# thiery-lab/manifold-mcmc-for-diffusions

Measured on AMD Instinct MI355X. Metric: constrained-leapfrog steps/sec (all chains), FHN noisy-obs 400 sub-steps, higher is better.
Workload: dtype f64; 1 GPU; FHN noisy-obs, T=100 obs, S=400 steps/obs, R=5 obs/subseq, sigma_y=0.1, 256 chains per GPU (BASELINE.json configs[1]), Newton solver, standard splitting; chains_per_gpu=256, global_chains=256, dim_q=80106, traj_len=16, stepping=chmc_leapfrog_steps per trajectory (batched steps), chain_steps_nominal=152320, parallelism=chains x1 (no data-path collective, 1 gather), ranks_joined=1, collective_world_size=1, collective_route=torch.distributed gather, overlap_halves=-1

## Files before the change

### manifold_mcmc_for_diffusions_amd/context.py

```python
import ctypes as C
import numpy as np
from . import _lib
from ._lib import ChmcConfig, as_c, ptr, iptr, check

MODEL_IDS = {"fhn": 0, "sir": 1, "fhn_nb": 2}
STATUS_NAMES = {0: "ok", 1: "not_converged", 2: "diverged", 3: "non_reversible", -1: "inactive"}


class ChmcContext:
    def __init__(self, model, obs_interval, num_steps_per_obs, num_obs_per_subseq, y_seq, sigma=None,
                 use_gaussian_splitting=False, num_chains=1, device=0):
        L = _lib.lib()
        self.L = L
        y = as_c(np.asarray(y_seq).reshape(-1))
        self._y = y
        cfg = ChmcConfig(
            model=MODEL_IDS[model] if isinstance(model, str) else int(model), num_obs=len(y),
            num_steps_per_obs=int(num_steps_per_obs),
            num_obs_per_subseq=0 if num_obs_per_subseq is None else int(num_obs_per_subseq),
            noisy=2 if isinstance(sigma, str) else int(sigma is not None),
            use_gaussian_splitting=int(bool(use_gaussian_splitting)),
            num_chains=int(num_chains), device=int(device), obs_interval=float(obs_interval),
            sigma=0.0 if sigma is None or isinstance(sigma, str) else float(sigma), y_seq=ptr(y))
        h = C.c_void_p()
# ... 317 lines not shown
                                         constraint_tol, position_tol, divergence_tol, int(max_iters), reverse_check_tol,
                                         iptr(ndone), iptr(status), iptr(itf), iptr(itb), ptr(rev)), "chmc_leapfrog_steps")
        return dict(n_done=ndone, status=status, iters_fwd=itf, iters_bwd=itb, rev_err=rev)

    def comm_init(self, id128, rank, world):
        buf = (C.c_char * 128).from_buffer_copy(bytes(id128))
        check(self.L.chmc_comm_init(self.h, buf, int(rank), int(world)), "chmc_comm_init")
        self.comm_world = int(world)

    @staticmethod
    def comm_unique_id():
        buf = (C.c_char * 128)()
        check(_lib.lib().chmc_comm_unique_id(buf), "chmc_comm_unique_id")
        return bytes(buf)

    def gather_samples_device(self, local_dev_ptr, count, gathered_dev_ptr):
        check(self.L.chmc_gather_samples(self.h, C.c_void_p(local_dev_ptr), int(count), C.c_void_p(gathered_dev_ptr)),
              "chmc_gather_samples")

    def comm_info(self):
        wd, rk = C.c_int(0), C.c_int(0)
        check(self.L.chmc_comm_info(self.h, C.byref(wd), C.byref(rk)), "chmc_comm_info")
        return wd.value, rk.value

    def comm_destroy(self):
        check(self.L.chmc_comm_destroy(self.h), "chmc_comm_destroy")

    def diagnostics(self):
        out = (C.c_longlong * 80)()
        check(self.L.chmc_get_diagnostics(self.h, out), "chmc_get_diagnostics")
        v = np.array(out[:], dtype=np.int64)
        return dict(par_scan=v[:64], gram_mfma_launches=int(v[64]), gram_valu_launches=int(v[65]),
                    retract_kernel_launches=int(v[66]), traj_kernel_launches=int(v[67]),
                    newton_fsm_launches=int(v[68]), newton_factor8_launches=int(v[69]), extra=v[68:80])

    def counters(self):
        out = (C.c_longlong * 8)()
        check(self.L.chmc_get_counters(self.h, out), "chmc_get_counters")
        keys = ("constr", "jacob_constr_blocks", "lu_jacob_product_blocks", "chol_gram_blocks",
                "grad_log_det_sqrt_gram", "leapfrog_step", "projection_iterations", "_")
        return dict(zip(keys, (int(v) for v in out)))
```

### manifold_mcmc_for_diffusions_amd/csrc/chmc_api.inc

```
#include <string>
#include <algorithm>
#include <vector>
#include <cstring>
#include <cstdio>
#include <cstdlib>
#include <cmath>
#include <thread>
#include <type_traits>
#include "../../include/chmc.h"
#include "chmc_plan.h"
#include "chmc_layout.h"

using namespace chmc;

static thread_local std::string g_err;
static int fail(const std::string& m) {
  g_err = m;
  return -1;
}
#include CHMC_BACKEND_HEADER

struct chmc_ctx : ChainView {
  std::thread::id owner = std::this_thread::get_id();
  chmc_config cfg;
// ... 572 lines not shown
    else
      launch_wave(k_jw_wave<RM>, (long)sy.B * sy.K, 6, sy, c->sl, c->w, which, vsel | 256);
#else
    launch(KJw<RM>{sy, c->sl, c->w, which, vsel | 256}, (long)sy.B * sy.K * RM, 6);
#endif
    launch(KSymBlk<M, RM>{sy, c->sl, c->w, which, 0}, (long)sy.B * sy.K, 9);
    CHMC_SOLVE_CHAIN(M, RM, 1, 1, sy, c->sl, c->w, which, 0, psel);
    if (compact) {
      CHMC_UPDATE_PB(1, which, 0, psel);
    } else {
      CHMC_UPDATE(1, sy, c->sl, c->w, which, 0, psel);
    }
  });
}

static void iteration_scan(chmc_ctx* c, int newton, int prev, int qsel, int fwd_guess, int use_nw) {
  const Sys& sy = c->sy;
  CHMC_DISPATCH(c, {
    if (newton) {
#ifdef CHMC_WAVE_KERNELS
      CHMC_FWD(prev ^ 1, qsel, use_nw, 2, fwd_guess);
#else
      (void)fwd_guess, (void)use_nw;
#endif
    } else {
      CHMC_FWD(prev ^ 1, qsel, use_nw, 0, fwd_guess);
    }
  });
}
static void iteration_after_scan(chmc_ctx* c, int newton, int prev, int qsel) {
  const Sys& sy = c->sy;
  const NewtonSweep sweep = part_plan(c).newton;
  const bool solved = newton && (sweep == NewtonIvlFsm || sweep == Newton16IvlCombFactor || sweep == Newton16IvlCombWg);
  CHMC_DISPATCH(c, {
    if (newton) {
#ifdef CHMC_WAVE_KERNELS
      const long nbk = (long)sy.B * sy.K;
      if constexpr (RM > 8) {
        switch (sweep) {
          case Newton16IvlCombWg:
            launch_blocks(k_newton_ivl<M>, nbk * sy.NOBS, 64, 1, sy, c->sl, c->w, prev, qsel);
            launch_blocks(k_newton_comb_wg<M, RM, CHMC_RETRACT_WAVES, false>, (long)sy.B, 64 * CHMC_RETRACT_WAVES, 1, sy,
                          c->sl, c->w, prev, qsel);
            break;
          case Newton16IvlCombFactor:
            launch_blocks(k_newton_ivl<M>, nbk * sy.NOBS, 64, 1, sy, c->sl, c->w, prev, qsel);
            launch_blocks(k_newton_comb<M, RM, false, true>, nbk, 64, 1, sy, c->sl, c->w, prev, qsel);
            break;
          case Newton16IvlComb:
            launch_blocks(k_newton_ivl<M>, nbk * sy.NOBS, 64, 1, sy, c->sl, c->w, prev, qsel);
            launch_blocks(k_newton_comb<M, RM>, nbk, 64, 1, sy, c->sl, c->w, prev, qsel);
            break;
          case Newton16LdsrowsGramMfma:
            launch_blocks(k_rev_wave_ldsrows<M, RM, 1>, nbk, 64, 1, sy, c->sl, c->w, prev, qsel);
            launch_blocks(k_gram_rows_mfma<RM>, nbk, 64, 1, sy, c->sl, c->w, prev, 1, qsel), c->diag[0]++;
            break;
          default:
            launch_blocks(k_rev_wave_ldsrows<M, RM, 1>, nbk, 64, 1, sy, c->sl, c->w, prev, qsel);
            launch_wave(k_gram_rows<RM, 4>, nbk * (RM / 4), 1, sy, c->sl, c->w, prev, 1, qsel), c->diag[1]++;
        }
        if (!solved) launch_blocks(k_newton_factor_wave<M, RM>, (nbk + 3) / 4, 64, 9, sy, c->sl, c->w, prev, qsel);
      } else {
        switch (sweep) {
          case NewtonIvlFsm:
          case NewtonIvlComb:
            launch_blocks(k_newton_ivl<M>, nbk * sy.NOBS, 64, 1, sy, c->sl, c->w, prev, qsel);
            launch_blocks(k_newton_comb<M, RM>, nbk, 64, 1, sy, c->sl, c->w, prev, qsel);
            break;
          case NewtonRevStoreGramMfma:
            launch_wave(k_rev_wave<M, RM, 1, false>, nbk, 1, sy, c->sl, c->w, prev, qsel);
            launch_blocks(k_gram_rows_mfma<RM>, nbk, 64, 1, sy, c->sl, c->w, prev, 1, qsel), c->diag[0]++;
            break;
          default:
            launch_wave(k_rev_wave<M, RM, 1>, nbk, 1, sy, c->sl, c->w, prev, qsel);
        }
        if (solved)
          launch_blocks(k_newton_fsm_wave<M, RM>, (long)sy.B, 64, 5, sy, c->sl, c->w, prev, qsel), c->diag[4]++;
        else
          launch(KNewtonFactor<M, RM>{sy, c->sl, c->w, prev}, nbk, 9), c->diag[5]++;
      }
#else
      launch(KNewtonBlk<M, RM>{sy, c->sl, c->w, prev, qsel}, (long)sy.B * sy.K, 1);
#endif
      if (!solved) CHMC_SOLVE_CHAIN(M, RM, 0, 0, sy, c->sl, c->w, prev, qsel, 0);
    } else {
      launch(KSymBlk<M, RM>{sy, c->sl, c->w, prev, 1}, (long)sy.B * sy.K, 9);
      CHMC_SOLVE_CHAIN(M, RM, 1, 0, sy, c->sl, c->w, prev, qsel, 0);
    }
#ifdef CHMC_WAVE_KERNELS
    if (c->plan.rows == RowsCompact) {
      if (!solved) launch(KMuF<RM, M::X, 0>{sy, c->sl, c->w, prev}, (long)sy.B * sy.K * sy.NOBS * M::X, 5);
      launch_colmax(KUpdatePB<RM, M::X, M::V, 0, 1>{sy, c->sl, c->w, prev, qsel, 0},
                    sy.T * sy.S + sy.V0 + (sy.noisy ? sy.T : 0), sy.B, 4);
    } else
#endif
    CHMC_UPDATE(0, sy, c->sl, c->w, prev, qsel, 0);
  });
}

static int retract_waves(const chmc_ctx* c, int newton, const void* views) {
  return chain_kernel_waves(c->plan, part_plan(c).retract_chain, c->sy.B, c->num_cus, newton != 0, views != nullptr);
}
static int traj_waves(const chmc_ctx* c, int n_inner, int newton) {
  const bool eligible = part_plan(c).traj_chain && n_inner == 1 && c->mom_tangent && c->halves == 1;
  return chain_kernel_waves(c->plan, eligible, c->sy.B, c->num_cus, newton != 0, false);
}
static int run_projection(chmc_ctx* c, int newton, int prev, int qsel, double ctol, double ptol, double dtol,
                          int max_iters, const ViewSave* views = nullptr, int count_dir = -1) {
  const Sys& sy = c->sy;
#ifdef CHMC_WAVE_KERNELS
  if (const int waves = retract_waves(c, newton, views)) {
    int* iters_dst = count_dir < 0 ? nullptr : (count_dir ? c->d_itb : c->d_itf);
    CHMC_DISPATCH(c, {
      if constexpr (RM == 16) {
        if (waves == 4)
          launch_blocks(k_retract_chain<M, RM, 4>, (long)sy.B, 256, 1, sy, c->sl, c->w, prev, qsel, ctol, ptol, dtol, max_iters,
                        iters_dst);
        else
          launch_blocks(k_retract_chain<M, RM, CHMC_RETRACT_WAVES>, (long)sy.B, 64 * CHMC_RETRACT_WAVES, 1, sy, c->sl, c->w, prev,
                        qsel, ctol, ptol, dtol, max_iters, iters_dst);
      }
    });
    c->counters[6]++;
    c->diag[2]++;
    return 0;
  }
#endif
  const int nh = views ? 2 : 1;
  auto enter = [&](int h) {
    if (views) set_half(c, *views, h);
  };
  for (int h = 0; h < nh; ++h) {
    enter(h);
    if (sy.B > 0) launch(KNewtonBegin{c->w}, sy.B);
  }
  int fwd_guess = 2;
#ifdef CHMC_WAVE_KERNELS
  const bool carry = c->plan.par_scan && sy.K == 1;
#else
  const bool carry = false;
#endif
  const int max_rounds = carry ? 12 * (max_iters + 1) : max_iters;
  auto iteration = [&](int poll_slot) {
    iteration_scan(c, newton, prev, qsel, fwd_guess, 1);
    iteration_after_scan(c, newton, prev, qsel);
    const KCheck chk{c->w, ctol, ptol, dtol, max_iters, sy.B, count_dir < 0 ? nullptr : (count_dir ? c->d_itb : c->d_itf),
                     c->round & 3};
    if (poll_slot >= 0) launch_publish(chk, sy.B, c->w.n_active + (c->round & 3), poll_slot);
    else launch(chk, sy.B);
  };
  bool done[2] = {false, nh == 1};
  for (int h = 0; h < nh; ++h) {
    enter(h);
    if (sy.B <= 0) done[h] = true;
  }
  int& expect = c->proj_rounds[prev & 1];
  int& stable = c->proj_stable[prev & 1];
  const bool predict = !views && stable >= 3 && expect >= 2;
  int rounds_done = 0;
  for (int it = 0; it < max_rounds && !(done[0] && done[1]); ++it) {
    if (predict && it >= expect && poll_end((it - 1) & 1) == 0) {
      done[0] = true;
      break;
    }
    for (int h = 0; h < nh; ++h) {
      if (done[h]) continue;
      enter(h);
      fwd_guess = it == 0 ? 2 : 1;
      c->round = it;
      iteration(it >= 1 ? 2 * h + (it & 1) : -1);
    }
    c->counters[6]++;
    if (it == 0) continue;
    bool all_empty = true;
    for (int h = 0; h < nh; ++h) {
      if (done[h]) continue;
      if (it >= 2 && poll_end(2 * h + ((it - 1) & 1)) == 0) {
        done[h] = true;
        continue;
      }
      all_empty = false;
      if (it + 1 >= max_rounds) poll_end(2 * h + (it & 1));
    }
    if (all_empty) c->counters[6]--;
    else rounds_done = it + 1;
  }
  if (!views) {
    if (predict && done[0] && rounds_done < expect) rounds_done = expect;
    stable = rounds_done == expect ? stable + 1 : 0;
    expect = rounds_done;
  }
  for (int h = 0; h < nh; ++h) {
    enter(h);
    if (sy.B > 0) launch(KNewtonEnd{c->w, count_dir < 0 ? nullptr : (count_dir ? c->d_itb : c->d_itf)}, sy.B);
  }
  c->round = 0;
  return 0;
}

static int check_ctx(const chmc_ctx* c, const char* fn) {
  if (!c) return fail(std::string(fn) + ": null context");
  if (c->owner != std::this_thread::get_id())
    return fail(std::string(fn) + ": a context must be driven by the host thread that created it");
  return 0;
}
#define CHMC_ENTER(fn)                 \
  if (check_ctx(ctx, fn)) return -1;   \
  refresh_plan(ctx);                   \
  use_stream(-1);                      \
  if (dev_set(ctx->cfg.device)) return fail(std::string(fn) + ": " + g_err);
#define CHMC_LEAVE(fn)                                                 \
  if (dev_sync()) return fail(std::string(fn) + ": " + g_err);        \
  return 0;

extern "C" int chmc_get_diagnostics(chmc_ctx* ctx, long long* out80) {
  CHMC_ENTER("chmc_get_diagnostics")
  if (!out80) return fail("chmc_get_diagnostics: null output");
  int ps[80];
  d2h(ps, ctx->w.nfallback, sizeof(ps));
  for (int i = 0; i < 64; ++i) out80[i] = ps[i];
  for (int i = 0; i < 16; ++i) out80[64 + i] = ctx->diag[i];
#ifdef CHMC_RETRACT_PROF
  for (int i = 4; i < 16; ++i) out80[64 + i] = ps[64 + i - 4];
#endif
  CHMC_LEAVE("chmc_get_diagnostics")
}

// ... 683 lines not shown
  } else {
    ctx->last_active_null = true;
  }
  if (n_inner > 1) ensure_array(ctx, ctx->d_q0), ensure_array(ctx, ctx->d_p0), ensure_array(ctx, ctx->d_ncommit);
#ifdef CHMC_WAVE_KERNELS
  if (const int waves = traj_waves(ctx, n_inner, newton)) {
    ensure_array(ctx, ctx->d_nsteps), ensure_array(ctx, ctx->d_ndone);
    if (n_steps_host) h2d(ctx->d_nsteps, n_steps_host, sizeof(int) * sy.B);
    begin_all(ctx, d_dt ? ctx->w.err : nullptr, d_active ? ctx->d_act : nullptr, 1.0);
    dev_zero(ctx->d_itf, sizeof(int) * sy.B), dev_zero(ctx->d_itb, sizeof(int) * sy.B);
    CHMC_DISPATCH(ctx, {
      if constexpr (RM == 16) {
        if (waves == 4)
          launch_blocks(k_traj_chain<M, RM, 4>, (long)sy.B, 256, 1, sy, ctx->sl, ctx->w,
                        n_steps_host ? ctx->d_nsteps : nullptr, n_steps_all, ctol, ptol, dtol, max_iters, rev_tol, ctx->d_itf,
                        ctx->d_itb, want_n_done ? ctx->d_ndone : nullptr);
        else
          launch_blocks(k_traj_chain<M, RM, CHMC_RETRACT_WAVES>, (long)sy.B, 64 * CHMC_RETRACT_WAVES, 1, sy, ctx->sl, ctx->w,
                        n_steps_host ? ctx->d_nsteps : nullptr, n_steps_all, ctol, ptol, dtol, max_iters, rev_tol, ctx->d_itf,
                        ctx->d_itb, want_n_done ? ctx->d_ndone : nullptr);
      }
    });
    ctx->rows_fresh = false;
    ctx->diag[3]++;
    const int ns = n_steps_host ? 1 : n_steps_all;
    ctx->counters[0] += ns, ctx->counters[1] += ns, ctx->counters[3] += ns, ctx->counters[4] += ns, ctx->counters[6] += 2 * ns;
    return 0;
  }
#endif
  const bool two = ctx->halves == 2;
  const ViewSave full = save_view(ctx);
  const int nh = two ? 2 : 1;
  const double kick = 0.5 * n_inner;
  auto enter = [&](int h) {
    if (two) set_half(ctx, full, h);
  };
  if (two) streams_fork();
  for (int h = 0; h < nh; ++h) {
    enter(h);
    begin_all(ctx, d_dt ? ctx->w.err : nullptr, d_active ? ctx->d_act : nullptr, 1.0 / n_inner);
    dev_zero(ctx->d_itf, sizeof(int) * sy.B), dev_zero(ctx->d_itb, sizeof(int) * sy.B);
    if (n_inner > 1) {
      dev_zero(ctx->d_ncommit, sizeof(int) * sy.B);
      launch(KGatherState{sy, ctx->sl, ctx->d_q0, ctx->d_p0}, (long)sy.B * sy.Q, 8);
    }
  }
  for (int i = 0; i < n_inner; ++i) {
    const bool last = i == n_inner - 1;
    for (int h = 0; h < nh; ++h) {
      enter(h);
      if (i > 0) {
        launch_rows(KFlow{sy, ctx->sl, ctx->w, 0, 0, 0, 1.0}, sy.Q, sy.B, 8);
      } else if (ctx->mom_tangent) {
        if (pending_kick) launch_rows(KKick2FlowPg{sy, ctx->sl, ctx->w, kick}, sy.Q, sy.B, 8);
        else launch_rows(KKickFlowPg{sy, ctx->sl, ctx->w, kick}, sy.Q, sy.B, 8);
      } else {
        launch(KKick{sy, ctx->sl, ctx->w, 0, 1, kick}, (long)sy.B * sy.Q, 8);
        project_momentum(ctx, 0, 3, 2);
        launch_rows(KFlow{sy, ctx->sl, ctx->w, 0, 0, 1, 1.0}, sy.Q, sy.B, 8);
      }
    }
    run_projection(ctx, newton, 0, 0, ctol, ptol, dtol, max_iters, two ? &full : nullptr, 0);
    for (int h = 0; h < nh; ++h) {
      enter(h);
      state_eval_core(ctx, 1, last, 3);
      const bool fix_in_jw = last && ctx->plan.mom_fix_in_jp;
      if (fix_in_jw)
        launch_rows(KMomFixEdges{KMomFixInitPg{sy, ctx->sl, ctx->w, 1}}, sy.U + sy.V0 + (sy.Q - sy.U - sy.NV), sy.B, 8);
      else
        launch_rows(KMomFixInitPg{sy, ctx->sl, ctx->w, 1}, sy.Q, sy.B, 8);
      const bool flow_in_update = last && ctx->plan.rev_flow_in_update;
      if (last)
        project_momentum_and_kick_direction(ctx, 1, false, fix_in_jw, flow_in_update);
      else
        project_momentum(ctx, 1, 0, 0);
      launch_rows(KFlow{sy, ctx->sl, ctx->w, 1, 1, 0, -1.0}, flow_in_update ? sy.U : sy.Q, sy.B, 8);
    }
    run_projection(ctx, newton, 1, 1, ctol, ptol, dtol, max_iters, two ? &full : nullptr, 1);
    for (int h = 0; h < nh; ++h) {
      enter(h);
      launch_colmax(KRevDiff{sy, ctx->sl, ctx->w}, (sy.Q + 1) / 2, sy.B, 8);
      launch(KRevCheck{ctx->w, rev_tol}, sy.B);
      if (last) {
        if (!skip_end_kick) launch_rows(KKickPg{sy, ctx->sl, ctx->w, 1, 0, kick}, sy.Q, sy.B, 8);
        launch(KCommit{ctx->sl, ctx->w}, sy.B);
      } else {
        launch(KCommitInner{ctx->sl, ctx->w, ctx->d_ncommit}, sy.B);
      }
    }
  }
  if (two) {
    restore_view(ctx, full);
    streams_join();
    const int extra = n_inner;
    ctx->counters[0] -= extra, ctx->counters[1] -= extra, ctx->counters[3] -= extra, ctx->counters[4] -= 1;
  }
  return 0;
}
static void step_finish(chmc_ctx* ctx, bool masked, int n_inner, int* status, int* iters_fwd, int* iters_bwd,
                        double* rev_err) {
  const Sys& sy = ctx->sy;
  bool any_failed = false;
  {
    const size_t nb = (size_t)sy.B * (sizeof(double) + 3 * sizeof(int));
    ctx->h_out.resize(nb);
    d2h(ctx->h_out.data(), ctx->d_out, nb);
    const unsigned char* h = ctx->h_out.data();
    if (rev_err) memcpy(rev_err, h, sizeof(double) * sy.B);
    h += sizeof(double) * sy.B;
    if (status) memcpy(status, h, sizeof(int) * sy.B);
    if (iters_fwd) memcpy(iters_fwd, h + sizeof(int) * sy.B, sizeof(int) * sy.B);
    if (iters_bwd) memcpy(iters_bwd, h + 2 * sizeof(int) * sy.B, sizeof(int) * sy.B);
    const int* st = reinterpret_cast<const int*>(h);
    for (int c = 0; c < sy.B; ++c) any_failed = any_failed || st[c] > 0;
// ... 352 lines not shown
```

### manifold_mcmc_for_diffusions_amd/csrc/chmc_core.h

```cpp
#pragma once
#include <math.h>
#include <stdint.h>
#include "chmc_model.h"

#define CHMC_FI __attribute__((always_inline))
#if defined(__HIPCC__)
#define CHMC_UNROLL _Pragma("unroll")
#define CHMC_UNROLL4 _Pragma("unroll 4")
#else
#define CHMC_UNROLL
#define CHMC_UNROLL4
#endif

namespace chmc {

#ifndef CHMC_FWD_DEPTH
#define CHMC_FWD_DEPTH 4
#endif
#define CHMC_Q_PAD 256
#define CHMC_TPAD 16

struct BlockDesc {
  int obs0, nobs, first, last;
  int row0, nrows, ny;
// ... 2021 lines not shown
      const double2_ a = *reinterpret_cast<const double2_*>(w.qb + i), b = *reinterpret_cast<const double2_*>(qs + i);
      const unsigned long long u = absbits(a.x - b.x), v = absbits(a.y - b.y);
      return u > v ? u : v;
    }
    unsigned long long r = absbits(w.qb[i] - qs[i]);
    if (col + 1 < sy.Q) {
      const unsigned long long v = absbits(w.qb[i + 1] - qs[i + 1]);
      r = v > r ? v : r;
    }
    return r;
  }
};
struct KRevCheck {
  Work w;
  double tol;
  CHMC_FI CHMC_HD void operator()(int c) const {
    if (!w.ok[c]) return;
    const double r = bitsd(w.rev[c]);
    if (!(r <= tol)) w.ok[c] = 0, w.status[c] = 3;
  }
};
struct KCommit {
  Slots sl;
  Work w;
  CHMC_FI CHMC_HD void operator()(int c) const {
    if (w.ok[c]) sl.cur[c] ^= 1;
  }
};
struct KBegin {
  Work w;
  const int* active;
  const double* dt;
  double scale;
  CHMC_HD void operator()(int c) const {
    w.ok[c] = active ? (active[c] != 0) : 1;
    w.status[c] = w.ok[c] ? 0 : -1;
    if (dt) {
      const double h = scale * dt[c];
      w.dt[c] = h;
      w.sdt[c] = sin(h);
      w.cdt[c] = cos(h);
    }
    w.rev[c] = 0ULL;
  }
};
struct KAddIters {
  Work w;
  int* dst;
  CHMC_HD void operator()(int c) const {
    if (w.ok[c] || w.status[c] > 0) dst[c] += w.iters[c];
  }
};
struct KCommitInner {
  Slots sl;
  Work w;
  int* ncommit;
  CHMC_HD void operator()(int c) const {
    if (w.ok[c]) {
      sl.cur[c] ^= 1;
      ncommit[c] += 1;
      w.rev[c] = 0ULL;
    }
  }
};
struct KCopyPadMasked {
  Work w;
  double* dst;
  const double* src;
  int n;
  CHMC_HD void operator()(int tid) const {
    if (w.ok[tid / n]) dst[tid] = src[tid];
  }
};

#define CHMC_TREE_MAXCHK 10
#define CHMC_ROWSUM_MAX (6 * CHMC_TREE_MAXCHK)
struct KTreeLeaf {
  Sys sy;
  Slots sl;
  const int* run;
  const int* take;
  double* sub_prop_q;
  double* sub_sum;
  double* ck_p;
  double* ck_sum;
  double* ck_end;
  int store, lo, nchk;
  CHMC_HD bool active(int c) const { return run[c] != 0; }
  CHMC_HD double2_ vel(const double* base, size_t cq, int col, double2_ p) const {
    if (sy.m0 && col < sy.U) {
      p.x = metric_inv_u(sy, base + cq, col);
      if (col + 1 < sy.U) p.y = metric_inv_u(sy, base + cq, col + 1);
    }
    return p;
  }
// ... 342 lines not shown
```

### manifold_mcmc_for_diffusions_amd/csrc/chmc_plan.h

```cpp
#pragma once
#include <climits>
#include <cstdlib>

#ifndef CHMC_RETRACT_WAVES
#define CHMC_RETRACT_WAVES 8
#endif
#ifndef CHMC_CHAIN_SCAN_WAVES
#define CHMC_CHAIN_SCAN_WAVES 4
#endif
#ifndef CHMC_CHAIN_WG4_MAX_PER_CU
#define CHMC_CHAIN_WG4_MAX_PER_CU 4
#endif

namespace chmc {

constexpr int kSwitchUnset = INT_MIN;
struct Switches {
  bool compact_rows = true, gram_mfma = false;
  int par_scan = kSwitchUnset, par_waves = kSwitchUnset, row_split = 0, halves = 1;
  bool no_fwd_scan = false, step_fusions = true;
  int retract_kernel = kSwitchUnset;
};
inline Switches read_switches() {
  auto env = [](const char* name, int unset) {
    const char* e = getenv(name);
    return e ? atoi(e) : unset;
  };
  static const bool compact_rows = env("CHMC_COMPACT_ROWS", 1) != 0, gram_mfma = env("CHMC_GRAM_MFMA", 0) != 0;
  Switches s;
  s.compact_rows = compact_rows, s.gram_mfma = gram_mfma;
  s.par_scan = env("CHMC_PAR_SCAN", kSwitchUnset), s.par_waves = env("CHMC_PAR_WAVES", kSwitchUnset);
  s.row_split = env("CHMC_ROW_SPLIT", 0), s.halves = env("CHMC_HALVES", 1);
  s.no_fwd_scan = getenv("CHMC_NO_FWD_SCAN") != nullptr, s.step_fusions = env("CHMC_STEP_FUSIONS", 1) != 0;
  s.retract_kernel = env("CHMC_RETRACT_KERNEL", kSwitchUnset);
  return s;
}

struct PlanInput {
  int rmt;
  int num_partition;
  int K[2];
  int longest;
  int chain_steps;
  bool s_tiles8;
  int V;
  bool even_dims;
  bool gaussian;
  bool wave_kernels;
  Switches sw;
  Switches call;
};

enum RowFamily { RowsCompact, RowsStored, RowsStoredMfma };
enum FwdScan { FwdPar , FwdWave , FwdFunctor  };
enum StateSweep {
  StateLean,
  StateIvlComb,
  StateIvlCombWg,
  StateLdsrowsGram,
  StateLdsrowsGramMfma,
  StateRevWave,
  StateRevStoreGramMfma
};
enum NewtonSweep {
  NewtonIvlFsm,
// ... 4 lines not shown
  Newton16IvlCombFactor,
  Newton16IvlComb,
  Newton16LdsrowsGram,
  Newton16LdsrowsGramMfma
};
enum GldSweep {
  GldQxLean,
  GldIvl,
  GldCompactFwdStored,
  GldStored
};
enum JpPass { JpPb , JpPbWg , JpWave  };

struct PartitionPlan {
  StateSweep state;
  NewtonSweep newton;
  GldSweep gld;
  JpPass jp;
  bool rebuild_rows;
  bool retract_chain;
  bool traj_chain;
};
struct KernelPlan {
  RowFamily rows;
  bool pb_allocated;
  bool par_scan;
  FwdScan fwd;
  FwdScan fwd_cold;
  int fwd_waves;
  FwdScan nld;
  int nld_waves;
  bool mom_fix_in_jp;
  bool rev_flow_in_update;
  int retract_kernel;
  PartitionPlan part[2];
};

inline int par_waves_for(int env, long longest) {
  if (env == 1 || env == 2 || env == 4) return env;
  return longest >= 4096 ? 4 : longest >= 2048 ? 2 : 1;
}
inline bool few_long_blocks(int nblocks_per_chain, long longest) { return nblocks_per_chain <= 4 && longest >= 1024; }

inline KernelPlan make_plan(const PlanInput& in) {
  const Switches& sw = in.sw;
  KernelPlan pl{};
  const bool rows16 = in.rmt > 8;
  const int kmax = in.K[0] > in.K[in.num_partition - 1] ? in.K[0] : in.K[in.num_partition - 1];
  const bool chain16_layout = kmax == 1 && rows16;

  const bool compact = in.wave_kernels && sw.compact_rows && !sw.gram_mfma;
  pl.rows = compact ? RowsCompact : sw.gram_mfma ? RowsStoredMfma : RowsStored;
  pl.pb_allocated = compact || (in.wave_kernels && sw.compact_rows && rows16);

  pl.par_scan = sw.par_scan != kSwitchUnset ? sw.par_scan != 0
                                            : few_long_blocks(kmax, in.longest) || (chain16_layout && sw.compact_rows && !sw.gram_mfma);
  pl.fwd_waves = chain16_layout && sw.par_waves == kSwitchUnset ? CHMC_CHAIN_SCAN_WAVES : par_waves_for(sw.par_waves, in.longest);
  pl.fwd_cold = in.wave_kernels && in.s_tiles8 && !in.call.no_fwd_scan ? FwdWave : FwdFunctor;
  pl.fwd = in.wave_kernels && pl.par_scan ? FwdPar : pl.fwd_cold;
  const bool nld_par = in.call.par_scan != kSwitchUnset ? in.call.par_scan != 0 : few_long_blocks(1, in.chain_steps);
  pl.nld = nld_par ? FwdPar : in.s_tiles8 ? FwdWave : FwdFunctor;
  pl.nld_waves = par_waves_for(in.call.par_waves, in.chain_steps);

  const bool step_fusions = pl.pb_allocated && in.call.step_fusions && !rows16;
  pl.mom_fix_in_jp = step_fusions && in.V == 2 && in.even_dims;
  pl.rev_flow_in_update = step_fusions && !in.gaussian;
  pl.retract_kernel = in.call.retract_kernel;

  for (int p = 0; p < in.num_partition; ++p) {
    PartitionPlan& pp = pl.part[p];
    const int K = in.K[p];
    const bool split = sw.row_split == 1 ? false : (sw.row_split == 2 || sw.row_split == 4) ? true : K <= 4;
    const bool ivl16 = rows16 && compact && split;
    const bool chain16 = chain16_layout && ivl16;
    if (rows16) {
      pp.state = chain16 ? StateIvlCombWg : ivl16 ? StateIvlComb : sw.gram_mfma ? StateLdsrowsGramMfma : StateLdsrowsGram;
      pp.newton = chain16 ? Newton16IvlCombWg
                  : compact ? (K == 1 ? Newton16IvlCombFactor : Newton16IvlComb)
                  : sw.gram_mfma ? Newton16LdsrowsGramMfma : Newton16LdsrowsGram;
      pp.gld = ivl16 ? GldIvl : compact ? GldCompactFwdStored : GldStored;
    } else {
      pp.state = compact ? StateLean : sw.gram_mfma ? StateRevStoreGramMfma : StateRevWave;
      pp.newton = compact ? (K <= 64 ? NewtonIvlFsm : NewtonIvlComb) : sw.gram_mfma ? NewtonRevStoreGramMfma : NewtonRevWave;
      pp.gld = compact ? GldQxLean : GldStored;
    }
    pp.jp = chain16 ? JpPbWg : compact ? JpPb : JpWave;
    pp.rebuild_rows = compact && (!rows16 || ivl16);
    pp.retract_chain = compact && rows16 && K == 1;
    pp.traj_chain = pp.retract_chain && ivl16;
  }
  return pl;
}

inline int chain_kernel_waves(const KernelPlan& pl, bool eligible, int B, int num_cus, bool newton, bool half_batches) {
  if (!eligible || !newton || half_batches) return 0;
  const int want = pl.retract_kernel != kSwitchUnset ? pl.retract_kernel
                   : B <= num_cus ? 1 : B <= CHMC_CHAIN_WG4_MAX_PER_CU * num_cus ? 2 : 0;
  return want == 1 ? CHMC_RETRACT_WAVES : want == 2 ? 4 : 0;
}
// ... 3 lines not shown
```

### manifold_mcmc_for_diffusions_amd/csrc/chmc_wave.h

```cpp
#pragma once
#include <type_traits>
#include "chmc_core.h"

namespace chmc {

#ifdef CHMC_PLAIN_STREAM
__device__ inline double ld_stream(const double* p) { return *p; }
#else
__device__ inline double ld_stream(const double* p) { return __builtin_nontemporal_load(p); }
#endif

__device__ __forceinline__ void st_async(double* p, double v) {
  asm volatile("global_store_dwordx2 %0, %1, off\n\ts_nop 1" : : "v"(p), "v"(v) : "memory");
}
__device__ __forceinline__ void st_async2(double* p, double v0, double v1) {
  typedef double d2v __attribute__((ext_vector_type(2)));
  const d2v v = {v0, v1};
  asm volatile("global_store_dwordx4 %0, %1, off\n\ts_nop 1" : : "v"(p), "v"(v) : "memory");
}

__device__ inline double bcast0(double x) {
  union { double d; int i[2]; } u;
  u.d = x;
  u.i[0] = __builtin_amdgcn_readfirstlane(u.i[0]);
// ... 1241 lines not shown
  double* out = w.ivl + (cb * sy.NOBS + m) * CHMC_IVL_N(X, Z);
#pragma unroll
  for (int i = 0; i < X * X; ++i) {
    double v = Sacc[i];
#pragma unroll
    for (int o = 32; o > 0; o >>= 1) v += __shfl_xor(v, o, 64);
    if (lane == 0) out[i] = v;
  }
#pragma unroll
  for (int i = 0; i < X * Z; ++i) {
    double v = Wacc[i];
#pragma unroll
    for (int o = 32; o > 0; o >>= 1) v += __shfl_xor(v, o, 64);
    if (lane == 0) out[X * X + i] = v;
  }
  if (lane == 0) {
#pragma unroll
    for (int i = 0; i < X * X; ++i) out[X * X + X * Z + i] = Pf[i];
  }
}
template <class M, bool STATE = false>
__global__ void __launch_bounds__(64, CHMC_IVL_WAVES) k_newton_ivl(Sys sy, Slots sl, Work w, int which, int qsel) {
  const int wid = blockIdx.x;
  if (wid >= sy.B * sy.K * sy.NOBS) return;
  const int m = wid % sy.NOBS;
  const int cbi = sy.order[wid / sy.NOBS];
  const int c = cbi / sy.K, b = cbi - c * sy.K;
  if (STATE ? !w.ok[c] : !newton_select(w, c, which, qsel)) return;
  const BlockDesc bd = sy.blk[b];
  if (m >= bd.nobs) return;
  newton_ivl_body<M, STATE>(sy, sl, w, which, qsel, c, b, m, bd);
}

template <class M, int RM, bool STATE, bool FACTOR>
__device__ __forceinline__ void newton_comb_body(const Sys& sy, const Slots& sl, const Work& w, int which, int qsel, int c, int b,
                                                 const BlockDesc& bd) {
  constexpr int X = M::X, Z = M::Z, U = M::U, V0 = M::V0;
  constexpr int NI = CHMC_IVL_N(X, Z);
  static_assert(!(STATE && FACTOR), "the factor step belongs to a Newton iteration");
  __shared__ double LamF[RM * X], LamN[RM * X], Dl[RM * RM], zl[RM * Z], Ys[RM * X], Iv[NI], JuS[FACTOR ? RM * M::U : 1];
  const int lane = threadIdx.x & 63;
  const int sl_ = sl.cur[c] ^ which;
  const size_t cb = (size_t)c * sy.Kmax + b;
  const int S = sy.S, NV = sy.NV;
  const double* q = (STATE ? pick(sl.q, sl_) : (qsel ? w.qb : pick(sl.q, sl_ ^ 1))) + (size_t)c * sy.Q;
  const double* traj = (STATE ? pick(sl.traj, sl_) : w.trajw) + (size_t)c * sy.TRJ + (size_t)(bd.step0 + CHMC_TPAD * b) * X;
  double* Jr = pick(sl.Jv, sl_) + (size_t)c * RM * NV;
  double* LFr = pick(sl.LF, sl_) + cb * sy.NOBS * RM * X;
  auto lds_sync = [&]() {
    __builtin_amdgcn_fence(__ATOMIC_ACQ_REL, "workgroup");
    __builtin_amdgcn_wave_barrier();
  };
  for (int e = lane; e < RM * X; e += 64) LamF[e] = 0.0;
  for (int e = lane; e < RM * RM; e += 64) Dl[e] = 0.0;
  for (int e = lane; e < RM * Z; e += 64) zl[e] = 0.0;
  lds_sync();
  for (int m = bd.nobs - 1; m >= 0; --m) {
    if (m < bd.ny) {
      double g[X], gl = 0.0;
      M::obs_grad(traj + (size_t)(m + 1) * S * X, g);
#pragma unroll
      for (int a = 0; a < X; ++a) gl = lane == a ? g[a] : gl;
      if (lane < X) LamF[m * X + lane] = gl;
    }
    if (m == bd.nobs - 1 && !bd.last) {
      if (lane < X) LamF[(bd.ny + lane) * X + lane] = 1.0;
    }
    const double* iv = w.ivl + (cb * sy.NOBS + m) * NI;
    for (int e = lane; e < NI; e += 64) Iv[e] = iv[e];
    lds_sync();
    if constexpr (STATE) {
      for (int e = lane; e < RM * X; e += 64) LFr[(size_t)m * RM * X + e] = LamF[e];
    }
// ... 37 lines not shown
    for (int e = lane; e < RM * RM; e += 64) {
      const int i = e / RM, jj = e - i * RM;
      double tt = Dl[e];
      for (int d = 0; d < V0; ++d) {
        double j0 = 0.0, j1 = 0.0;
        for (int a = 0; a < X; ++a) j0 += LamF[i * X + a] * dv0[a * V0 + d], j1 += LamF[jj * X + a] * dv0[a * V0 + d];
        tt += j0 * (STATE ? j1 : Jr[(size_t)jj * NV + d]);
        if (STATE && jj == 0) Jr[(size_t)i * NV + d] = j0;
      }
      Dl[e] = tt;
    }
    for (int e = lane; e < RM * Z; e += 64) {
      const int i = e / Z, mz = e - i * Z;
      double tt = zl[e];
      for (int a = 0; a < X; ++a) {
        double dzs = 0.0;
#pragma unroll
        for (int ee = 0; ee < X * Z; ++ee) dzs = ee == a * Z + mz ? dz[ee] : dzs;
        tt += LamF[i * X + a] * dzs;
      }
      zl[e] = tt;
    }
  }
  lds_sync();
  for (int e = lane; e < RM * RM; e += 64) {
    const int i = e / RM, jj = e - i * RM;
    double v = Dl[e];
    if (i == jj) {
      const double sg_ = sy.noisy ? sigma_at(sy, q) : 0.0;
      if (sy.noisy && i < bd.ny) v += sg_ * sigma_at(sy, pick(sl.q, sl_) + (size_t)c * sy.Q);
      if (i >= bd.nrows) v = 1.0;
    }
    if constexpr (FACTOR) Dl[e] = v;
    else w.Dw[cb * RM * RM + e] = v;
  }
  double G[Z * Z];
  M::gz_jac(q, G);
  for (int e = lane; e < RM * U; e += 64) {
    const int i = e / U, d = e - i * U;
    double tt = 0.0;
    if (d < Z) {
      for (int mz = 0; mz < Z; ++mz) {
        double gs = 0.0;
#pragma unroll
        for (int ee = 0; ee < Z * Z; ++ee) gs = ee == mz * Z + d ? G[ee] : gs;
        tt += zl[i * Z + mz] * gs;
      }
    } else {
      tt = i < bd.ny ? sigma_at(sy, q) * q[sy.U + sy.NV + bd.obs0 + i] : 0.0;
    }
    if constexpr (FACTOR) JuS[e] = tt;
    else (STATE ? pick(sl.JuP, sl_) : w.JuL)[cb * RM * U + e] = tt;
  }
  if constexpr (STATE) {
    for (int e = lane; e < RM * Z; e += 64) w.zbP[cb * RM * Z + e] = zl[e];
  }
  if constexpr (FACTOR) {
    lds_sync();
    newton_factor16<M, RM, true>(sy, sl, w, which, qsel, c, b, lane < 16, Dl, JuS);
  }
}
template <class M, int RM, bool STATE = false, bool FACTOR = false>
__global__ void __launch_bounds__(64) k_newton_comb(Sys sy, Slots sl, Work w, int which, int qsel) {
  const int wid = blockIdx.x;
  if (wid >= sy.B * sy.K) return;
  const int cbi = sy.order[wid];
  const int c = cbi / sy.K, b = cbi - c * sy.K;
  if (STATE ? !w.ok[c] : !newton_select(w, c, which, qsel)) return;
  const BlockDesc bd = sy.blk[b];
  newton_comb_body<M, RM, STATE, FACTOR>(sy, sl, w, which, qsel, c, b, bd);
}

template <class M, int RM, int MODE>
__global__ void __launch_bounds__(64) k_rev_wave_ldsrows(Sys sy, Slots sl, Work w, int which, int qsel) {
  constexpr int X = M::X, V = M::V, Z = M::Z, U = M::U, V0 = M::V0;
  __shared__ double LamS[RM * X];
  __shared__ double zaccS[RM * Z * 64];
  const int lane = threadIdx.x & 63;
  const int wid = blockIdx.x;
  if (wid >= sy.B * sy.K) return;
  const int cbi = sy.order[wid];
  const int c = cbi / sy.K, b = cbi - c * sy.K;
  if (MODE == 1 ? !newton_select(w, c, which, qsel) : !w.ok[c]) return;
  const BlockDesc bd = sy.blk[b];
// ... 2597 lines not shown
    double t = x[i];
#pragma unroll
    for (int k = 0; k < RM; ++k)
      if (k > i) t -= L[k * RM + i] * x[k];
    x[i] = t / L[i * RM + i];
  }
  if (!act) return;
#pragma unroll
  for (int i = 0; i < RM; ++i) {
    double t = 0.0;
#pragma unroll
    for (int a = 0; a < U; ++a) t += Ws[g][i * U + a] * e[a];
    const double v = (i >= nrows || r >= nrows) ? 0.0 : x[i] - t;
    w.gMb[cb * RM * RM + i * RM + r] = v;
  }
  double Gz[Z * Z];
  M::gz_jac(pick(sl.q, s) + (size_t)c * sy.Q, Gz);
#pragma unroll
  for (int d = 0; d < U; ++d) w.gWu[(cb * RM + r) * U + d] = wu[d];
#pragma unroll
  for (int mz = 0; mz < Z; ++mz) {
    double t = 0.0;
#pragma unroll
    for (int d = 0; d < Z; ++d) t += Gz[mz * Z + d] * wu[d];
    w.gzd[(cb * RM + r) * Z + mz] = t;
  }
}
template <class M, int RM>
__global__ void __launch_bounds__(64) k_gld_prep_wave(Sys sy, Slots sl, Work w, int which) {
  gld_prep_body<M, RM>(sy, sl, w, which, blockIdx.x * 4, 4);
}


template <class M, int RM>
__global__ void __launch_bounds__(64) k_newton_fsm_wave(Sys sy, Slots sl, Work w, int prev, int qsel) {
  constexpr int U = M::U, X = M::X;
  static_assert(RM <= 8, "one block per lane: the RM x RM matrix lives in registers");
  const int lane = threadIdx.x & 63;
  const int c = blockIdx.x;
  if (c >= sy.B) return;
  if (!newton_select(w, c, prev, qsel)) return;
  const int sp = sl.cur[c] ^ prev;
  const bool has = lane < sy.K;
  const size_t cb = (size_t)c * sy.Kmax + (has ? lane : 0);
  double D[RM * RM], JuL[RM * U], cp[RM];
  unsigned long long eb = 0ULL;
#pragma unroll
  for (int i = 0; i < RM * RM; ++i) D[i] = has ? w.Dw[cb * RM * RM + i] : ((i / RM == i % RM) ? 1.0 : 0.0);
#pragma unroll
  for (int i = 0; i < RM * U; ++i) JuL[i] = has ? w.JuL[cb * RM * U + i] : 0.0;
#pragma unroll
  for (int i = 0; i < RM; ++i) {
    cp[i] = has ? w.cpad[cb * RM + i] : 0.0;
    const unsigned long long vb = absbits(cp[i]);
    eb = vb > eb ? vb : eb;
  }
  {
    int piv[RM];
    lu_factor<RM>(D, piv);
    lu_solve<RM, 1>(D, piv, cp);
    lu_solve<RM, U>(D, piv, JuL);
  }
  const double* jur = pick(sl.JuP, sp) + cb * RM * U;
  double ju[RM * U];
#pragma unroll
  for (int i = 0; i < RM * U; ++i) ju[i] = has ? jur[i] : 0.0;
  double sacc[U], Cm[U * U];
#pragma unroll
  for (int a = 0; a < U; ++a) {
    double t2 = 0.0;
#pragma unroll
    for (int i = 0; i < RM; ++i) t2 += ju[i * U + a] * cp[i];
    sacc[a] = has ? t2 : 0.0;
#pragma unroll
    for (int d = 0; d < U; ++d) {
      double t = 0.0;
#pragma unroll
      for (int i = 0; i < RM; ++i) t += ju[i * U + a] * JuL[i * U + d];
      Cm[a * U + d] = has ? t : 0.0;
    }
  }
#pragma unroll
  for (int a = 0; a < U; ++a) {
// ... 56 lines not shown
    const BlockDesc bd = sy.blk[lane];
    const double* lfb = pick(sl.LF, sp) + cb * sy.NOBS * RM * X;
    double* mo = w.muF + cb * sy.NOBS * X;
    for (int m0 = 0; m0 < sy.NOBS; m0 += 4) {
      double t4[4][X], lf[4][RM * X];
#pragma unroll
      for (int k = 0; k < 4; ++k) {
        const bool in = m0 + k < sy.NOBS;
#pragma unroll
        for (int e = 0; e < RM * X; ++e) lf[k][e] = in ? lfb[(m0 + k) * RM * X + e] : 0.0;
      }
#pragma unroll
      for (int k = 0; k < 4; ++k) {
        const int m = m0 + k;
#pragma unroll
        for (int a = 0; a < X; ++a) {
          double t = 0.0;
          if (m < bd.nobs) {
#pragma unroll
            for (int i = 0; i < RM; ++i)
              if (i < bd.nrows) t += lam[i] * lf[k][i * X + a];
          }
          t4[k][a] = t;
        }
      }
#pragma unroll
      for (int k = 0; k < 4; ++k)
        if (m0 + k < sy.NOBS) {
#pragma unroll
          for (int a = 0; a < X; ++a) mo[(m0 + k) * X + a] = t4[k][a];
        }
    }
  }
}

template <class M, int RM, bool FUSE = false>
__global__ void __launch_bounds__(64) k_newton_factor_wave(Sys sy, Slots sl, Work w, int prev, int qsel) {
  const int lane = threadIdx.x & 63;
  const int tid = blockIdx.x * 4 + (lane >> 4);
  const bool live = tid < sy.B * sy.K;
  const int tc = live ? tid : 0;
  const int c = tc / sy.K, b = tc - c * sy.K;
  const bool act = newton_select(w, c, prev, qsel) && live;
  const size_t cb = (size_t)c * sy.Kmax + b;
  newton_factor16<M, RM, FUSE>(sy, sl, w, prev, qsel, c, b, act, w.Dw + cb * RM * RM, w.JuL + cb * RM * M::U);
}

typedef double d2_t __attribute__((ext_vector_type(2)));
template <int OFF>
__device__ __forceinline__ void vm_load16(d2_t& dst, const void* p) {
  asm volatile("global_load_dwordx4 %0, %1, off offset:%2" : "=v"(dst) : "v"(p), "n"(OFF) : "memory");
}
template <int I, int N, int OFF0>
struct TileLoad {
  static __device__ __forceinline__ void run(d2_t* r, const void* p) {
    vm_load16<OFF0 + 16 * I>(r[I], p);
    TileLoad<I + 1, N, OFF0>::run(r, p);
  }
};
template <int N, int OFF0>
struct TileLoad<N, N, OFF0> {
  static __device__ __forceinline__ void run(d2_t*, const void*) {}
};
template <int NOUT>
__device__ __forceinline__ void vm_wait(d2_t (&r)[8]) {
  asm volatile("s_waitcnt vmcnt(%8)"
// ... 805 lines not shown
```

Measured before the change: 52750 steps/s.

## Fuse per-chain begin/end bookkeeping kernels and add workgroup Newton round kernel

Adds a chain_fusions plan switch, on by default for compact non-rows16 layouts. With it, the step-begin bookkeeping, the iteration-counter zeroing and the Newton-begin reset run as one per-chain kernel. The Newton-end, reversibility check and commit at step end also collapse into a single KStepEnd launch, removing several tiny launches per leapfrog step. An opt-in (chain_fusions>=2) workgroup kernel also computes the Newton combine for all blocks into LDS and runs the FSM solve in the same launch, avoiding a global round-trip of the D and Ju matrices. The fused path reorders commit relative to the final kick, so it must select the right state slot.

```diff
diff --git a/manifold_mcmc_for_diffusions_amd/context.py b/manifold_mcmc_for_diffusions_amd/context.py
--- a/manifold_mcmc_for_diffusions_amd/context.py
+++ b/manifold_mcmc_for_diffusions_amd/context.py
@@ -373,7 +373,8 @@
         v = np.array(out[:], dtype=np.int64)
         return dict(par_scan=v[:64], gram_mfma_launches=int(v[64]), gram_valu_launches=int(v[65]),
                     retract_kernel_launches=int(v[66]), traj_kernel_launches=int(v[67]),
-                    newton_fsm_launches=int(v[68]), newton_factor8_launches=int(v[69]), extra=v[68:80])
+                    newton_fsm_launches=int(v[68]), newton_factor8_launches=int(v[69]),
+                    newton_round_launches=int(v[70]), step_end_launches=int(v[71]), extra=v[68:80])
 
     def counters(self):
         out = (C.c_longlong * 8)()
diff --git a/manifold_mcmc_for_diffusions_amd/csrc/chmc_api.inc b/manifold_mcmc_for_diffusions_amd/csrc/chmc_api.inc
--- a/manifold_mcmc_for_diffusions_amd/csrc/chmc_api.inc
+++ b/manifold_mcmc_for_diffusions_amd/csrc/chmc_api.inc
@@ -628,6 +628,8 @@
   const Sys& sy = c->sy;
   const NewtonSweep sweep = part_plan(c).newton;
   const bool solved = newton && (sweep == NewtonIvlFsm || sweep == Newton16IvlCombFactor || sweep == Newton16IvlCombWg);
+  const bool round_wg = solved && sweep == NewtonIvlFsm && c->plan.chain_fusions >= 2 && sy.K <= CHMC_ROUND_MAX_BLOCKS;
+  (void)round_wg;
   CHMC_DISPATCH(c, {
     if (newton) {
 #ifdef CHMC_WAVE_KERNELS
@@ -661,7 +663,11 @@
           case NewtonIvlFsm:
           case NewtonIvlComb:
             launch_blocks(k_newton_ivl<M>, nbk * sy.NOBS, 64, 1, sy, c->sl, c->w, prev, qsel);
-            launch_blocks(k_newton_comb<M, RM>, nbk, 64, 1, sy, c->sl, c->w, prev, qsel);
+            if (round_wg)
+              launch_blocks(k_newton_round_wg<M, RM, CHMC_ROUND_WAVES>, (long)sy.B, 64 * CHMC_ROUND_WAVES, 1, sy, c->sl, c->w,
+                            prev, qsel), c->diag[6]++;
+            else
+              launch_blocks(k_newton_comb<M, RM>, nbk, 64, 1, sy, c->sl, c->w, prev, qsel);
             break;
           case NewtonRevStoreGramMfma:
             launch_wave(k_rev_wave<M, RM, 1, false>, nbk, 1, sy, c->sl, c->w, prev, qsel);
@@ -670,7 +676,8 @@
           default:
             launch_wave(k_rev_wave<M, RM, 1>, nbk, 1, sy, c->sl, c->w, prev, qsel);
         }
-        if (solved)
+        if (round_wg) {
+        } else if (solved)
           launch_blocks(k_newton_fsm_wave<M, RM>, (long)sy.B, 64, 5, sy, c->sl, c->w, prev, qsel), c->diag[4]++;
         else
           launch(KNewtonFactor<M, RM>{sy, c->sl, c->w, prev}, nbk, 9), c->diag[5]++;
@@ -702,7 +709,8 @@
   return chain_kernel_waves(c->plan, eligible, c->sy.B, c->num_cus, newton != 0, false);
 }
 static int run_projection(chmc_ctx* c, int newton, int prev, int qsel, double ctol, double ptol, double dtol,
-                          int max_iters, const ViewSave* views = nullptr, int count_dir = -1) {
+                          int max_iters, const ViewSave* views = nullptr, int count_dir = -1, bool begun = false,
+                          bool end_later = false) {
   const Sys& sy = c->sy;
 #ifdef CHMC_WAVE_KERNELS
   if (const int waves = retract_waves(c, newton, views)) {
@@ -728,7 +736,7 @@
   };
   for (int h = 0; h < nh; ++h) {
     enter(h);
-    if (sy.B > 0) launch(KNewtonBegin{c->w}, sy.B);
+    if (sy.B > 0 && !begun) launch(KNewtonBegin{c->w}, sy.B);
   }
   int fwd_guess = 2;
 #ifdef CHMC_WAVE_KERNELS
@@ -788,7 +796,7 @@
   }
   for (int h = 0; h < nh; ++h) {
     enter(h);
-    if (sy.B > 0) launch(KNewtonEnd{c->w, count_dir < 0 ? nullptr : (count_dir ? c->d_itb : c->d_itf)}, sy.B);
+    if (sy.B > 0 && !end_later) launch(KNewtonEnd{c->w, count_dir < 0 ? nullptr : (count_dir ? c->d_itb : c->d_itf)}, sy.B);
   }
   c->round = 0;
   return 0;
@@ -1538,14 +1546,20 @@
   const ViewSave full = save_view(ctx);
   const int nh = two ? 2 : 1;
   const double kick = 0.5 * n_inner;
+  const bool chain_fusions = ctx->plan.chain_fusions != 0;
   auto enter = [&](int h) {
     if (two) set_half(ctx, full, h);
   };
   if (two) streams_fork();
   for (int h = 0; h < nh; ++h) {
     enter(h);
-    begin_all(ctx, d_dt ? ctx->w.err : nullptr, d_active ? ctx->d_act : nullptr, 1.0 / n_inner);
-    dev_zero(ctx->d_itf, sizeof(int) * sy.B), dev_zero(ctx->d_itb, sizeof(int) * sy.B);
+    if (chain_fusions) {
+      launch(KBegin{ctx->w, d_active ? ctx->d_act : nullptr, d_dt ? ctx->w.err : nullptr, 1.0 / n_inner, ctx->d_itf, ctx->d_itb,
+                    true}, sy.B);
+    } else {
+      begin_all(ctx, d_dt ? ctx->w.err : nullptr, d_active ? ctx->d_act : nullptr, 1.0 / n_inner);
+      dev_zero(ctx->d_itf, sizeof(int) * sy.B), dev_zero(ctx->d_itb, sizeof(int) * sy.B);
+    }
     if (n_inner > 1) {
       dev_zero(ctx->d_ncommit, sizeof(int) * sy.B);
       launch(KGatherState{sy, ctx->sl, ctx->d_q0, ctx->d_p0}, (long)sy.B * sy.Q, 8);
@@ -1566,7 +1580,7 @@
         launch_rows(KFlow{sy, ctx->sl, ctx->w, 0, 0, 1, 1.0}, sy.Q, sy.B, 8);
       }
     }
-    run_projection(ctx, newton, 0, 0, ctol, ptol, dtol, max_iters, two ? &full : nullptr, 0);
+    run_projection(ctx, newton, 0, 0, ctol, ptol, dtol, max_iters, two ? &full : nullptr, 0, chain_fusions && i == 0);
     for (int h = 0; h < nh; ++h) {
       enter(h);
       state_eval_core(ctx, 1, last, 3);
@@ -1582,10 +1596,15 @@
         project_momentum(ctx, 1, 0, 0);
       launch_rows(KFlow{sy, ctx->sl, ctx->w, 1, 1, 0, -1.0}, flow_in_update ? sy.U : sy.Q, sy.B, 8);
     }
-    run_projection(ctx, newton, 1, 1, ctol, ptol, dtol, max_iters, two ? &full : nullptr, 1);
+    run_projection(ctx, newton, 1, 1, ctol, ptol, dtol, max_iters, two ? &full : nullptr, 1, false, chain_fusions);
     for (int h = 0; h < nh; ++h) {
       enter(h);
       launch_colmax(KRevDiff{sy, ctx->sl, ctx->w}, (sy.Q + 1) / 2, sy.B, 8);
+      if (chain_fusions) {
+        launch(KStepEnd{ctx->sl, ctx->w, ctx->d_itb, rev_tol, last ? nullptr : ctx->d_ncommit}, sy.B), ctx->diag[7]++;
+        if (last && !skip_end_kick) launch_rows(KKickPg{sy, ctx->sl, ctx->w, 0, 0, kick}, sy.Q, sy.B, 8);
+        continue;
+      }
       launch(KRevCheck{ctx->w, rev_tol}, sy.B);
       if (last) {
         if (!skip_end_kick) launch_rows(KKickPg{sy, ctx->sl, ctx->w, 1, 0, kick}, sy.Q, sy.B, 8);
diff --git a/manifold_mcmc_for_diffusions_amd/csrc/chmc_core.h b/manifold_mcmc_for_diffusions_amd/csrc/chmc_core.h
--- a/manifold_mcmc_for_diffusions_amd/csrc/chmc_core.h
+++ b/manifold_mcmc_for_diffusions_amd/csrc/chmc_core.h
@@ -2077,6 +2077,8 @@
   const int* active;
   const double* dt;
   double scale;
+  int *itf = nullptr, *itb = nullptr;
+  bool newton_begin = false;
   CHMC_HD void operator()(int c) const {
     w.ok[c] = active ? (active[c] != 0) : 1;
     w.status[c] = w.ok[c] ? 0 : -1;
@@ -2087,6 +2089,8 @@
       w.cdt[c] = cos(h);
     }
     w.rev[c] = 0ULL;
+    if (itf) itf[c] = 0, itb[c] = 0;
+    if (newton_begin) KNewtonBegin{w}(c);
   }
 };
 struct KAddIters {
@@ -2106,6 +2110,22 @@
       ncommit[c] += 1;
       w.rev[c] = 0ULL;
     }
+  }
+};
+struct KStepEnd {
+  Slots sl;
+  Work w;
+  int* iters_dst;
+  double tol;
+  int* ncommit;
+  CHMC_HD void operator()(int c) const {
+    if (w.nw[c]) {
+      KNewtonEnd{w, iters_dst}(c);
+      w.rev[c] = 0ULL;
+    }
+    KRevCheck{w, tol}(c);
+    if (ncommit) KCommitInner{sl, w, ncommit}(c);
+    else KCommit{sl, w}(c);
   }
 };
 struct KCopyPadMasked {
diff --git a/manifold_mcmc_for_diffusions_amd/csrc/chmc_plan.h b/manifold_mcmc_for_diffusions_amd/csrc/chmc_plan.h
--- a/manifold_mcmc_for_diffusions_amd/csrc/chmc_plan.h
+++ b/manifold_mcmc_for_diffusions_amd/csrc/chmc_plan.h
@@ -7,6 +7,12 @@
 #endif
 #ifndef CHMC_CHAIN_SCAN_WAVES
 #define CHMC_CHAIN_SCAN_WAVES 4
+#endif
+#ifndef CHMC_ROUND_WAVES
+#define CHMC_ROUND_WAVES 4
+#endif
+#ifndef CHMC_ROUND_MAX_BLOCKS
+#define CHMC_ROUND_MAX_BLOCKS 32
 #endif
 #ifndef CHMC_CHAIN_WG4_MAX_PER_CU
 #define CHMC_CHAIN_WG4_MAX_PER_CU 4
@@ -19,6 +25,7 @@
   bool compact_rows = true, gram_mfma = false;
   int par_scan = kSwitchUnset, par_waves = kSwitchUnset, row_split = 0, halves = 1;
   bool no_fwd_scan = false, step_fusions = true;
+  int chain_fusions = 1;
   int retract_kernel = kSwitchUnset;
 };
 inline Switches read_switches() {
@@ -31,6 +38,7 @@
   s.compact_rows = compact_rows, s.gram_mfma = gram_mfma;
   s.par_scan = env("CHMC_PAR_SCAN", kSwitchUnset), s.par_waves = env("CHMC_PAR_WAVES", kSwitchUnset);
   s.row_split = env("CHMC_ROW_SPLIT", 0), s.halves = env("CHMC_HALVES", 1);
+  s.chain_fusions = env("CHMC_CHAIN_FUSIONS", 1);
   s.no_fwd_scan = getenv("CHMC_NO_FWD_SCAN") != nullptr, s.step_fusions = env("CHMC_STEP_FUSIONS", 1) != 0;
   s.retract_kernel = env("CHMC_RETRACT_KERNEL", kSwitchUnset);
   return s;
@@ -101,6 +109,7 @@
   int nld_waves;
   bool mom_fix_in_jp;
   bool rev_flow_in_update;
+  int chain_fusions;
   int retract_kernel;
   PartitionPlan part[2];
 };
@@ -134,6 +143,7 @@
   const bool step_fusions = pl.pb_allocated && in.call.step_fusions && !rows16;
   pl.mom_fix_in_jp = step_fusions && in.V == 2 && in.even_dims;
   pl.rev_flow_in_update = step_fusions && !in.gaussian;
+  pl.chain_fusions = compact && !rows16 ? (sw.chain_fusions >= 2 ? 2 : sw.chain_fusions == 1 ? 1 : 0) : 0;
   pl.retract_kernel = in.call.retract_kernel;
 
   for (int p = 0; p < in.num_partition; ++p) {
diff --git a/manifold_mcmc_for_diffusions_amd/csrc/chmc_wave.h b/manifold_mcmc_for_diffusions_amd/csrc/chmc_wave.h
--- a/manifold_mcmc_for_diffusions_amd/csrc/chmc_wave.h
+++ b/manifold_mcmc_for_diffusions_amd/csrc/chmc_wave.h
@@ -1297,13 +1297,19 @@
   newton_ivl_body<M, STATE>(sy, sl, w, which, qsel, c, b, m, bd);
 }
 
-template <class M, int RM, bool STATE, bool FACTOR>
+template <class M, int RM, bool STATE, bool FACTOR, int NW = 1, bool LDSOUT = false>
 __device__ __forceinline__ void newton_comb_body(const Sys& sy, const Slots& sl, const Work& w, int which, int qsel, int c, int b,
-                                                 const BlockDesc& bd) {
+                                                 const BlockDesc& bd, double* Dout = nullptr, double* Jout = nullptr) {
   constexpr int X = M::X, Z = M::Z, U = M::U, V0 = M::V0;
   constexpr int NI = CHMC_IVL_N(X, Z);
   static_assert(!(STATE && FACTOR), "the factor step belongs to a Newton iteration");
-  __shared__ double LamF[RM * X], LamN[RM * X], Dl[RM * RM], zl[RM * Z], Ys[RM * X], Iv[NI], JuS[FACTOR ? RM * M::U : 1];
+  static_assert(!LDSOUT || !(STATE || FACTOR), "LDS outputs: the Newton combine only");
+  __shared__ double LamF_[NW][RM * X], LamN_[NW][RM * X], Dl_[NW][RM * RM], zl_[NW][RM * Z], Ys_[NW][RM * X], Iv_[NW][NI],
+      JuS_[NW][FACTOR ? RM * M::U : 1];
+  const int wv_ = NW > 1 ? __builtin_amdgcn_readfirstlane(threadIdx.x >> 6) : 0;
+  double *const LamF = LamF_[wv_], *const LamN = LamN_[wv_], *const Dl = Dl_[wv_], *const zl = zl_[wv_], *const Ys = Ys_[wv_],
+                *const Iv = Iv_[wv_], *const JuS = JuS_[wv_];
+  (void)JuS, (void)Dout, (void)Jout;
   const int lane = threadIdx.x & 63;
   const int sl_ = sl.cur[c] ^ which;
   const size_t cb = (size_t)c * sy.Kmax + b;
@@ -1407,6 +1413,7 @@
       if (i >= bd.nrows) v = 1.0;
     }
     if constexpr (FACTOR) Dl[e] = v;
+    else if constexpr (LDSOUT) Dout[e] = v;
     else w.Dw[cb * RM * RM + e] = v;
   }
   double G[Z * Z];
@@ -1425,6 +1432,7 @@
       tt = i < bd.ny ? sigma_at(sy, q) * q[sy.U + sy.NV + bd.obs0 + i] : 0.0;
     }
     if constexpr (FACTOR) JuS[e] = tt;
+    else if constexpr (LDSOUT) Jout[e] = tt;
     else (STATE ? pick(sl.JuP, sl_) : w.JuL)[cb * RM * U + e] = tt;
   }
   if constexpr (STATE) {
@@ -4088,23 +4096,32 @@
 }
 
 
-template <class M, int RM>
-__global__ void __launch_bounds__(64) k_newton_fsm_wave(Sys sy, Slots sl, Work w, int prev, int qsel) {
+#define CHMC_ROUND_DSTRIDE(RM_) ((RM_) * (RM_) + 1)
+#define CHMC_ROUND_JSTRIDE(RM_, U_) ((RM_) * (U_) + 1)
+template <class M, int RM, bool LDSIN>
+__device__ __forceinline__ void newton_fsm_body(const Sys& sy, const Slots& sl, const Work& w, int prev, int qsel, int c,
+                                                const double* Dsrc, const double* Jsrc) {
   constexpr int U = M::U, X = M::X;
   static_assert(RM <= 8, "one block per lane: the RM x RM matrix lives in registers");
   const int lane = threadIdx.x & 63;
-  const int c = blockIdx.x;
-  if (c >= sy.B) return;
-  if (!newton_select(w, c, prev, qsel)) return;
   const int sp = sl.cur[c] ^ prev;
   const bool has = lane < sy.K;
   const size_t cb = (size_t)c * sy.Kmax + (has ? lane : 0);
   double D[RM * RM], JuL[RM * U], cp[RM];
   unsigned long long eb = 0ULL;
-#pragma unroll
-  for (int i = 0; i < RM * RM; ++i) D[i] = has ? w.Dw[cb * RM * RM + i] : ((i / RM == i % RM) ? 1.0 : 0.0);
-#pragma unroll
-  for (int i = 0; i < RM * U; ++i) JuL[i] = has ? w.JuL[cb * RM * U + i] : 0.0;
+  if constexpr (LDSIN) {
+    const double* dl = Dsrc + (has ? lane : 0) * CHMC_ROUND_DSTRIDE(RM);
+    const double* jl = Jsrc + (has ? lane : 0) * CHMC_ROUND_JSTRIDE(RM, U);
+#pragma unroll
+    for (int i = 0; i < RM * RM; ++i) D[i] = has ? dl[i] : ((i / RM == i % RM) ? 1.0 : 0.0);
+#pragma unroll
+    for (int i = 0; i < RM * U; ++i) JuL[i] = has ? jl[i] : 0.0;
+  } else {
+#pragma unroll
+    for (int i = 0; i < RM * RM; ++i) D[i] = has ? w.Dw[cb * RM * RM + i] : ((i / RM == i % RM) ? 1.0 : 0.0);
+#pragma unroll
+    for (int i = 0; i < RM * U; ++i) JuL[i] = has ? w.JuL[cb * RM * U + i] : 0.0;
+  }
 #pragma unroll
   for (int i = 0; i < RM; ++i) {
     cp[i] = has ? w.cpad[cb * RM + i] : 0.0;
@@ -4227,6 +4244,34 @@
         }
     }
   }
+}
+template <class M, int RM>
+__global__ void __launch_bounds__(64) k_newton_fsm_wave(Sys sy, Slots sl, Work w, int prev, int qsel) {
+  const int c = blockIdx.x;
+  if (c >= sy.B) return;
+  if (!newton_select(w, c, prev, qsel)) return;
+  newton_fsm_body<M, RM, false>(sy, sl, w, prev, qsel, c, nullptr, nullptr);
+}
+
+#ifndef CHMC_ROUND_MAX_BLOCKS
+#define CHMC_ROUND_MAX_BLOCKS 32
+#endif
+template <class M, int RM, int NW>
+__global__ void __launch_bounds__(64 * NW) k_newton_round_wg(Sys sy, Slots sl, Work w, int prev, int qsel) {
+  constexpr int U = M::U;
+  __shared__ double Dsh[CHMC_ROUND_MAX_BLOCKS * CHMC_ROUND_DSTRIDE(RM)], Jsh[CHMC_ROUND_MAX_BLOCKS * CHMC_ROUND_JSTRIDE(RM, U)];
+  const int c = blockIdx.x;
+  if (c >= sy.B || sy.K > CHMC_ROUND_MAX_BLOCKS) return;
+  if (!newton_select(w, c, prev, qsel)) return;
+  const int wv = __builtin_amdgcn_readfirstlane(threadIdx.x >> 6);
+  for (int b = wv; b < sy.K; b += NW) {
+    newton_comb_body<M, RM, false, false, NW, true>(sy, sl, w, prev, qsel, c, b, sy.blk[b], Dsh + b * CHMC_ROUND_DSTRIDE(RM),
+                                                    Jsh + b * CHMC_ROUND_JSTRIDE(RM, U));
+    __builtin_amdgcn_fence(__ATOMIC_ACQ_REL, "workgroup");
+    __builtin_amdgcn_wave_barrier();
+  }
+  __syncthreads();
+  if (wv == 0) newton_fsm_body<M, RM, true>(sy, sl, w, prev, qsel, c, Dsh, Jsh);
 }
 
 template <class M, int RM, bool FUSE = false>
```

Measured after the change: 53020 steps/s, median of 6. About the same (+0.5%).
